# tensorflow/compression

Hardware: AMD Instinct MI355X
Metric: Mpixels/s encode+decode round-trip (bit-exact) (higher is better)
Workload: dtype int32

## Files before the change

### compression_amd/_lib.py

```python
from __future__ import annotations

import ctypes as C
import os

_HERE = os.path.dirname(os.path.abspath(__file__))
LIB_PATH = os.path.join(_HERE, "libtfc_hip.so")

_vp = C.c_void_p
_i64 = C.c_int64
_int = C.c_int

SIGNATURES = {
    "tfc_abi_version": (_int, []),
    "tfc_last_error": (C.c_char_p, []),
    "tfc_profile_enable": (None, [_int]),
    "tfc_set_default_mode": (_int, [_int]),
    "tfc_get_default_mode": (_int, []),
    "tfc_set_chip_shared": (_int, [_int]),
    "tfc_image_to_unit": (_int, [_vp, _vp, _int, C.c_int64, _vp]),
    "tfc_unit_to_image": (_int, [_vp, _int, _vp, C.c_int64, _vp]),
    "tfc_index_prepare": (_int, [_vp, _int, _vp, C.c_int64, _int, _vp]),
    "tfc_build_tables": (_int, [_vp, C.c_int64, C.c_int64, _vp, _vp, C.c_int64, _int, _vp, _vp]),
    "tfc_build_tables_overflow": (_int, [_vp, C.c_int64, C.c_int64, _vp, _vp, C.c_int64, _int, _vp, _vp, _vp]),
    "tfc_deep_factorized_tails": (_int, [_vp, C.c_int64, C.c_int64, _int, _int, _vp, _int, _vp, _vp, _vp]),
    "tfc_pad2d": (_int, [_vp, _vp, _int, C.c_int64, C.c_int64, C.c_int64, C.c_int64, _int, _int, _int, _int, _int, _vp]),
    "tfc_cache_bytes": (_int, [C.POINTER(C.c_longlong)]),
    "tfc_cache_trim": (_int, [C.POINTER(C.c_longlong)]),
    "tfc_encoder_capacity": (_int, [_vp, C.POINTER(_i64)]),
    "tfc_profile_query": (_int, [C.c_char_p, C.POINTER(C.c_double), C.POINTER(_i64)]),
    "tfc_pipe_counters": (_int, [C.POINTER(_i64), C.POINTER(_i64)]),
    "tfc_set_pipe_format": (_int, [_int, _int]),
    "tfc_tables_create": (_int, [_vp, _int, _i64, _i64, _vp, C.POINTER(_vp)]),
    "tfc_tables_count": (_i64, [_vp]),
    "tfc_tables_destroy": (None, [_vp]),
    "tfc_encoder_create": (_int, [_vp, _i64, _vp, C.POINTER(_vp)]),
    "tfc_encoder_create_many": (_int, [_vp, _i64, _int, _vp, _vp]),
    "tfc_encoder_set_mode": (_int, [_vp, _int]),
    "tfc_encoder_set_deferred_errors": (_int, [_vp, _int]),
    "tfc_encoder_encode": (_int, [_vp, _vp, _vp, _i64, _vp]),
    "tfc_encoder_encode_many": (_int, [_int, _vp, _vp, _vp, _i64, _vp]),
    "tfc_encoder_encode_quantized": (_int, [_vp, _vp, _int, _vp, _vp, _i64, _i64, _vp]),
    "tfc_encoder_encode_quantized_indexed": (_int, [_vp, _vp, _int, _vp, _vp, _i64, _vp]),
    "tfc_encoder_encode_quantized_many": (_int, [_int, _vp, _vp, _int, _vp, _vp, _i64, _i64, _vp]),
    "tfc_decoder_decode_dequantized_many": (_int, [_int, _vp, _vp, _int, _vp, _vp, _i64, _i64, _vp]),
    "tfc_encoder_encode_quantized_indexed_many": (_int, [_int, _vp, _vp, _int, _vp, _vp, _i64, _vp]),
    "tfc_decoder_decode_dequantized_indexed_many": (_int, [_int, _vp, _vp, _vp, _int, _vp, _i64, _vp]),
    "tfc_encoder_finalize": (_int, [_vp, _vp, C.POINTER(_i64)]),
    "tfc_encoder_finalize_device": (_int, [_vp, _vp]),
    "tfc_encoder_finalize_device_many": (_int, [_int, _vp, _vp]),
    "tfc_encoder_status": (_int, [_vp, _vp, C.POINTER(_i64)]),
    "tfc_encoder_result": (_int, [_vp, C.POINTER(_vp), C.POINTER(_vp)]),
    "tfc_encoder_read": (_int, [_vp, _vp, _vp, _int, _vp]),
    "tfc_encoder_destroy": (None, [_vp]),
    "tfc_decoder_create": (_int, [_vp, _vp, _vp, _i64, _int, _vp, C.POINTER(_vp)]),
    "tfc_decoder_create_many": (_int, [_vp, _int, _vp, _vp, _vp]),
    "tfc_decoder_set_mode": (_int, [_vp, _int]),
    "tfc_decoder_decode": (_int, [_vp, _vp, _vp, _i64, _vp]),
    "tfc_decoder_decode_many": (_int, [_int, _vp, _vp, _vp, _i64, _vp]),
    "tfc_decoder_decode_dequantized": (_int, [_vp, _vp, _vp, _int, _vp, _vp, _i64, _i64, _vp]),
    "tfc_decoder_finalize": (_int, [_vp, _vp, _vp]),
    "tfc_decoder_finalize_device": (_int, [_vp, _vp, _vp]),
    "tfc_decoder_finalize_device_many": (_int, [_int, _vp, _vp, _vp]),
    "tfc_decoder_status": (_int, [_vp, _vp]),
    "tfc_decoder_destroy": (None, [_vp]),
# ... 139 lines not shown
```

### compression_amd/csrc/range_coder.hip

```cpp
#include <hip/hip_bf16.h>
#include <hip/hip_fp16.h>
#include <hip/hip_runtime.h>

#include <algorithm>
#include <atomic>
#include <cstdlib>
#include <cstring>
#include <type_traits>
#include <memory>
#include <mutex>
#include <string>
#include <vector>

#include "../../include/tfc_hip.h"
#include "common.h"
#include "range_coder_device.h"
#include "range_tables.h"
#include "range_wave.h"

using namespace tfc;


namespace tfc {

// ... 530 lines not shown
  }
}
__global__ void fill_state_kernel(uint4* state, int64_t n, uint4 v, unsigned long long* status,
                                  unsigned int* oflag) {
  fill_state_one(state, n, v, status, oflag);
}
__global__ void fill_state_many_kernel(uint8_t* ctl, long long ctl_bytes, int64_t n, uint4 v) {
  uint8_t* c = ctl + blockIdx.y * ctl_bytes;
  fill_state_one(reinterpret_cast<uint4*>(c + 64), n, v, reinterpret_cast<unsigned long long*>(c),
                 reinterpret_cast<unsigned int*>(c + 32));
}

}


namespace {

int env_int(const char* name, int fallback) {
  const char* e = std::getenv(name);
  return e ? std::atoi(e) : fallback;
}

std::atomic<int>& pipe_format_value() {
  static std::atomic<int> v{[] {
    const char* e = std::getenv("TFC_PIPE_FORMAT");
    if (e && std::strcmp(e, "full") == 0) return 1;
    if (e && std::strcmp(e, "pairs") == 0) return 2;
    return 0;
  }()};
  return v;
}
std::atomic<int>& pipe_waves_value() {
  static std::atomic<int> v{std::max(0, env_int("TFC_PIPE_WAVES", 0))};
  return v;
}
inline int pipe_format() { return pipe_format_value().load(std::memory_order_relaxed); }
inline int pipe_waves_env() { return pipe_waves_value().load(std::memory_order_relaxed); }

inline bool pipe_enabled() {
  static const bool on = env_int("TFC_PIPE", 1) != 0;
  return on;
}
inline bool pipe_fallback_launch() {
  static const bool on = env_int("TFC_PIPE_NOFALLBACK", 0) == 0;
  return on;
}
std::atomic<long long>& pipe_launches() {
  static std::atomic<long long> n{0};
  return n;
}

inline int pipe_overlap() {
  static const int v = env_int("TFC_PIPE_OVERLAP", 2);
  return v;
}
inline long long pipe_poll_ticks() {
  static const long long v = static_cast<long long>(env_int("TFC_PIPE_POLL_MS", 250)) * 100000;
  return v;
}

struct SideStream {
  hipStream_t stream = nullptr;
  hipEvent_t fork = nullptr, join = nullptr;
};
inline int side_stream(hipStream_t st, SideStream* out) {
  static std::mutex mu;
// ... 233 lines not shown
    for (int k = 0; k < gn; ++k) {
      tfc_encoder* e = es[g0 + k];
      e->elems_last = elems;
      e->indexed_last = indexed;
      if (speculative && !e->deferred) {
        TFC_HIP(backups[g0 + k].alloc(sizeof(uint4) * streams, st));
        TFC_HIP(hipMemcpyAsync(backups[g0 + k].p, e->state.p, sizeof(uint4) * streams, hipMemcpyDeviceToDevice, st));
      }
      EncChunk ch;
      ch.stride = la.cap;
      ch.data_bytes = static_cast<size_t>(la.cap) * streams;
      TFC_HIP(ch.data.alloc(ch.data_bytes + sizeof(unsigned int) * streams, st));
      ch.len_p = reinterpret_cast<unsigned int*>(ch.data.as<uint8_t>() + ch.data_bytes);
      EncLaneJob<Src>& J = jobs.job[k];
      J.src = srcs[g0 + k];
      J.index = indexed ? indexes[g0 + k] : nullptr;
      J.state = e->state.as<uint4>();
      J.chunk = ch.data.as<uint8_t>();
      J.chunk_len = ch.len_p;
      J.first_error = e->status.as<unsigned long long>();
      J.overflow_flag = e->oflag.as<unsigned int>();
      errs.job[k].status = J.first_error;
      errs.job[k].src = J.src;
      errs.job[k].index = J.index;
      e->chunks.push_back(std::move(ch));
    }
    {
      KernelTimer timer("enc_kernel", st);
      DevBuf temp;
      bool piped = pipe;
      la.guard = nullptr;
      if (pipe) do {
        const size_t groups = static_cast<size_t>(pa.groups_per_job) * gn;
        const size_t calls_bytes = (groups * 64 * pa.rows + 64 * PipeEncChainLds::kRows) * sizeof(unsigned int);
        const size_t stage_bytes = groups * 64 * (sizeof(uint4) + sizeof(uint2));
        const size_t status_bytes = groups * pa.nt * 64 * sizeof(unsigned int);
        const size_t done_bytes = (groups * pa.nt * sizeof(unsigned int) + 255) & ~size_t{255};
        if (temp.alloc(calls_bytes + stage_bytes + status_bytes + done_bytes + 512, st) != hipSuccess) {
          (void)hipGetLastError();
          temp.p = nullptr;
          piped = false;
          break;
        }
        uint8_t* base = temp.as<uint8_t>();
        pa.calls = reinterpret_cast<unsigned int*>(base);
        pa.stage_state = reinterpret_cast<uint4*>(base + calls_bytes);
        pa.stage_out = reinterpret_cast<uint2*>(base + calls_bytes + groups * 64 * sizeof(uint4));
        pa.status = reinterpret_cast<unsigned int*>(base + calls_bytes + stage_bytes);
        pa.done = reinterpret_cast<unsigned int*>(base + calls_bytes + stage_bytes + status_bytes);
        pa.fallback = reinterpret_cast<unsigned int*>(base + calls_bytes + stage_bytes + status_bytes + done_bytes);
        pa.started = pa.fallback + 64;
        pa.groups = static_cast<int>(groups);
        pipe_launches().fetch_add(1, std::memory_order_relaxed);
        pa.fast16 = t->d_fast.as<uint16_t>();
        pa.rows_fast = t->d_rows_fast.as<int2>();
        pa.ntab = la.ntab;
        pa.tab_entries = t->host.size() * 2 <= static_cast<size_t>(kExpandTabBytes) ? static_cast<int>(t->host.size()) : 0;
        pa.cap = la.cap;
        TFC_HIP(hipMemsetAsync(pa.status, 0, status_bytes + done_bytes + 512, st));
        PipeChainJobs cj;
        cj.streams = streams;
        for (int k = 0; k < gn; ++k)
          cj.job[k] = PipeChainJob{jobs.job[k].state, jobs.job[k].chunk, jobs.job[k].chunk_len, jobs.job[k].overflow_flag};
        const bool large = groups >= 64;
        const int overlap = large ? pipe_overlap() : 0;
        SideStream side;
        if (overlap) {
          if (side_stream(st, &side)) return 1;
          TFC_HIP(hipEventRecord(side.fork, st));
          TFC_HIP(hipStreamWaitEvent(side.stream, side.fork, 0));
        }
        const hipStream_t cst = overlap ? side.stream : st;
        const dim3 xgrid(static_cast<unsigned>(groups * pa.nt));
        auto expand = [&] {
          KernelTimer t2("enc_expand", st);
          const bool tlds = pa.tab_entries != 0;
          if (indexed && tlds) hipLaunchKernelGGL((enc_expand_kernel<true, Src, true>), xgrid, dim3(kExpandThreads), 0, st, jobs, pa);
          else if (indexed) hipLaunchKernelGGL((enc_expand_kernel<true, Src, false>), xgrid, dim3(kExpandThreads), 0, st, jobs, pa);
          else if (tlds) hipLaunchKernelGGL((enc_expand_kernel<false, Src, true>), xgrid, dim3(kExpandThreads), 0, st, jobs, pa);
          else hipLaunchKernelGGL((enc_expand_kernel<false, Src, false>), xgrid, dim3(kExpandThreads), 0, st, jobs, pa);
        };
        const int cgroups = PipeEncChainLds::kGroups;
        const unsigned cblocks = static_cast<unsigned>(ceil_div(static_cast<int64_t>(groups), cgroups));
        const int clds = cgroups * PipeEncChainLds::kGroup;
        if (large)
          TFC_HIP(hipFuncSetAttribute(reinterpret_cast<const void*>(&enc_chain_kernel), hipFuncAttributeMaxDynamicSharedMemorySize, clds));
        auto chain = [&] {
          KernelTimer t2("enc_chain", cst);
          if (!large) {
            hipLaunchKernelGGL(enc_chain_direct_kernel, dim3(static_cast<unsigned>(groups)), dim3(64), 0, cst, cj, pa);
            return;
          }
          hipLaunchKernelGGL(enc_chain_kernel, dim3(cblocks), dim3(256 * cgroups), clds, cst, cj, pa);
          if (overlap == 2)
            hipLaunchKernelGGL(enc_gate_kernel, dim3(1), dim3(1), 0, st, pa.started, cblocks, static_cast<long long>(20000));
        };
        if (overlap == 2) { chain(); expand(); }
        else { expand(); chain(); }
        if (overlap) {
          TFC_HIP(hipEventRecord(side.join, side.stream));
          TFC_HIP(hipStreamWaitEvent(st, side.join, 0));
        }
        hipLaunchKernelGGL(enc_commit_kernel, dim3(static_cast<unsigned>(groups)), dim3(64), 0, st, cj, pa);
        la.guard = pa.fallback;
      } while (false);
      const dim3 grid(static_cast<unsigned>(jobs.blocks_per_job * gn));
      if (piped && !pipe_fallback_launch()) {}
      else if (indexed) hipLaunchKernelGGL((enc_lanes_kernel<true, Src>), grid, dim3(block), lds_bytes, st, jobs, la);
      else hipLaunchKernelGGL((enc_lanes_kernel<false, Src>), grid, dim3(block), lds_bytes, st, jobs, la);
    }
    hipLaunchKernelGGL((enc_error_kernel<Src>), dim3(1), dim3(64), 0, st, errs);
    TFC_HIP(hipGetLastError());
  }
  bool any_eager = false;
  for (int k = 0; k < n; ++k) any_eager |= !es[k]->deferred;
  if (any_eager) {
    TFC_HIP(hipStreamSynchronize(st));
    for (int k = 0; k < n; ++k) {
      tfc_encoder* e = es[k];
      if (e->deferred) continue;
      unsigned long long host_status[4];
      TFC_HIP(hipMemcpy(host_status, e->status.p, sizeof(host_status), hipMemcpyDeviceToHost));
      if (host_status[0] != ~0ull) return encoder_error(e, host_status);
      if (!speculative) continue;
      unsigned int oflag = 0;
      TFC_HIP(hipMemcpy(&oflag, e->oflag.p, sizeof(oflag), hipMemcpyDeviceToHost));
// ... 378 lines not shown
  for (int k = 0; k < n; ++k) {
    tfc_encoder* e = es[k];
    e->result_group = group;
    e->offsets.p = f.base + k * f.job_bytes + f.offsets_off;
    e->blob.p = f.base + k * f.job_bytes + f.blob_off;
    e->blob_capacity = static_cast<int64_t>(cap);
    e->chunks.clear();
    e->finalized = true;
  }
  return 0;
}

extern "C" int tfc_debug_pipe_clocks(unsigned long long* out8) {
  TFC_HIP(hipDeviceSynchronize());
  TFC_HIP(hipMemcpyFromSymbol(out8, HIP_SYMBOL(tfc::g_pipe_clock), 8 * sizeof(unsigned long long)));
  return 0;
}
extern "C" int tfc_debug_enc_clocks(unsigned long long* out4) {
  TFC_HIP(hipDeviceSynchronize());
  TFC_HIP(hipMemcpyFromSymbol(out4, HIP_SYMBOL(tfc::g_enc_clock), 4 * sizeof(unsigned long long)));
  return 0;
}

extern "C" int tfc_pipe_counters(int64_t* launches, int64_t* fallback_blocks) {
  if (launches) *launches = pipe_launches().load();
  if (fallback_blocks) {
    unsigned long long v = 0;
    TFC_HIP(hipDeviceSynchronize());
    TFC_HIP(hipMemcpyFromSymbol(&v, HIP_SYMBOL(tfc::g_pipe_fallback_blocks), sizeof(v)));
    *fallback_blocks = static_cast<int64_t>(v);
  }
  return 0;
}

extern "C" int tfc_set_pipe_format(int format, int waves_per_workgroup) {
  if (format < 0 || format > 2 || waves_per_workgroup < 0 || waves_per_workgroup > 8) {
    tfc::fail("tfc_set_pipe_format: format 0 ... 2, waves per workgroup 0 ... 8");
    return -1;
  }
  pipe_waves_value().store(waves_per_workgroup);
  return pipe_format_value().exchange(format);
}

extern "C" int tfc_encoder_set_mode(tfc_encoder* e, int mode) {
  if (mode != TFC_MODE_AUTO && mode != TFC_MODE_LATENCY && mode != TFC_MODE_THROUGHPUT)
    return fail("unknown mode %d", mode);
  if (e->family >= 0) return fail("the mode of a handle is fixed by its first coding call");
  e->mode = mode;
  return 0;
}

extern "C" int tfc_encoder_set_deferred_errors(tfc_encoder* e, int on) {
  e->deferred = on != 0;
  return 0;
}

extern "C" int tfc_encoder_encode(tfc_encoder* e, const int32_t* value, const int32_t* index,
                                  int64_t elems, void* stream) {
  const SymInt32 src{value};
  return encode_jobs(&e, 1, &src, &index, elems, static_cast<hipStream_t>(stream), "tfc_encoder_encode");
}

extern "C" int tfc_encoder_encode_many(int n, tfc_encoder* const* es, const int32_t* const* values,
                                       const int32_t* const* indexes, int64_t elems, void* stream) {
  if (n <= 0) return 0;
  std::vector<SymInt32> srcs(n);
// ... 722 lines not shown
```

### compression_amd/csrc/range_pipe.h

```cpp
#pragma once

#ifndef TFC_PIPE_TIMING
#define TFC_PIPE_TIMING 0
#endif

namespace tfc {

constexpr int kPipeTile = 256;
constexpr int kPipeEscMax = 32;
constexpr unsigned int kPipeBlock = 16;
constexpr unsigned int kPipeNoCall = 0x0001FFFFu;
constexpr unsigned int kPipeAggregate = 1u << 30;
constexpr unsigned int kPipePrefix = 2u << 30;
constexpr unsigned int kPipeRowsMask = (1u << 30) - 1u;

struct PipeEncArgs {
  const uint16_t* fast16;
  const int2* rows_fast;
  int ntab;
  int tab_entries;
  unsigned int* calls;
  unsigned int* status;
  unsigned int* done;
  unsigned int* fallback;
  unsigned int* started;
  uint4* stage_state;
  uint2* stage_out;
  int nt;
  int rows;
  int groups_per_job;
  int groups;
  unsigned int cap;
  long long poll_ticks;
};


__device__ inline unsigned int pipe_escape_extra(unsigned int g) { return 2u * static_cast<unsigned int>(31 - __clz(static_cast<int>(g))) + 2u; }
__device__ inline unsigned int pipe_escape_word(unsigned int g, unsigned int neg, unsigned int extra, unsigned int k) {
  const unsigned int left = extra - k;
  const unsigned int sft = left - 1u;
  const unsigned int bit = left == 0u ? neg : (sft < 32u ? (g >> sft) & 1u : 0u);
  return bit ? 0x00008000u : 0x80000000u;
}

constexpr int kExpandThreads = 512;
constexpr int kExpandTabBytes = 32 * 1024;
template <bool INDEXED, typename Src, bool TABLDS>
__global__ void __launch_bounds__(kExpandThreads, 4) enc_expand_kernel(const EncLaneJobs<Src> jobs, const PipeEncArgs pa) {
  constexpr int kRow = kPipeTile;
  constexpr int kHalves = kExpandThreads / kPipeTile;
  __shared__ unsigned short W[64 * kRow];
  __shared__ __attribute__((aligned(16))) unsigned short tab[kExpandTabBytes / 2];
  __shared__ unsigned int esc[64][kPipeEscMax];
  __shared__ unsigned short ecum[64][kPipeEscMax];
  __shared__ unsigned int ecount[64], nesc[64], start[64];

  const unsigned int gi = blockIdx.x % static_cast<unsigned int>(pa.groups);
  const unsigned int T = blockIdx.x / static_cast<unsigned int>(pa.groups);
  const unsigned int job = gi / static_cast<unsigned int>(pa.groups_per_job);
  const unsigned int gidx = gi % static_cast<unsigned int>(pa.groups_per_job);
  const EncLaneJob<Src>& J = jobs.job[job];
  const Src src = J.src;
  const int32_t* const index = J.index;
  const unsigned int tid = threadIdx.x, lane = tid & 63u;
  const unsigned int elems = static_cast<unsigned int>(jobs.elems);
  const int64_t s0 = static_cast<int64_t>(gidx) * 64;
  const unsigned int ntab = static_cast<unsigned int>(pa.ntab);
  if (tid < 64u) ecount[tid] = 0u;
  constexpr bool tab_lds = TABLDS;
  if (tab_lds) {
    const uint4* const src16 = reinterpret_cast<const uint4*>(pa.fast16);
    for (unsigned int i = tid; i < (static_cast<unsigned int>(pa.tab_entries) + 7u) / 8u; i += kExpandThreads)
      reinterpret_cast<uint4*>(tab)[i] = src16[i];
  }
  __syncthreads();

  auto escape_of = [&](int64_t s, unsigned int at, unsigned int& g, unsigned int& neg) {
    const int64_t pos = s * jobs.elems + at;
    int t = static_cast<int>(at % ntab);
    if (INDEXED) {
      t = tfc_gload(index + pos);
      if (t < 0 || t >= pa.ntab) t = 0;
    }
    const int2 row = pa.rows_fast[t];
    const int32_t v = src.load(pos, t);
    const int32_t vmax = (row.y & 0x7FFFFFFF) - 3;
    neg = v < 0 ? 1u : 0u;
    g = v < 0 ? 0u - static_cast<unsigned int>(v) : static_cast<unsigned int>(v - vmax) + 1u;
  };

  {
    constexpr int N = 64 / kHalves;
    constexpr int NB = INDEXED ? 8 : 16;
    const unsigned int p = tid % kPipeTile, half = tid / kPipeTile;
    const unsigned int j = T * kPipeTile + p;
    const bool inpos = j < elems;
    const unsigned int jc = inpos ? j : 0u;
    const int tch = static_cast<int>(jc % ntab);
    const int2 rowc = pa.rows_fast[tch];
    unsigned long long badpos = ~0ull;
    auto position = [&](int i) {
      const int64_t s = s0 + i * kHalves + static_cast<int>(half);
// ... 80 lines not shown
    __hip_atomic_store(st + static_cast<size_t>(T) * 64, kPipeAggregate | cnt, __ATOMIC_RELAXED, __HIP_MEMORY_SCOPE_AGENT);
    unsigned int before = 0u;
    bool stuck = false;
    long long t0 = 0;
    for (unsigned int t = T; t-- > 0u && !stuck;) {
      unsigned int v, spins = 0u;
      while (((v = __hip_atomic_load(st + static_cast<size_t>(t) * 64, __ATOMIC_RELAXED, __HIP_MEMORY_SCOPE_AGENT)) >> 30) == 0u) {
        if (++spins < 64u) continue;
        __builtin_amdgcn_s_sleep(16);
        const long long now = static_cast<long long>(wall_clock64());
        if (t0 == 0) t0 = now;
        else if (now - t0 > pa.poll_ticks) { stuck = true; break; }
      }
      if (stuck) break;
      before += v & kPipeRowsMask;
      if (v & kPipePrefix) break;
    }
    const unsigned int limit = static_cast<unsigned int>(pa.rows);
    const bool fits = !stuck && before + cnt <= limit;
    if (!fits) atomicOr(&pa.fallback[job], 1u);
    __hip_atomic_store(st + static_cast<size_t>(T) * 64, kPipePrefix | (fits ? before + cnt : limit + 1u), __ATOMIC_RELAXED,
                       __HIP_MEMORY_SCOPE_AGENT);
    start[tid] = fits ? before : 0xFFFFFFFFu;
  }
  __syncthreads();

  {
    constexpr unsigned int kWaves = kExpandThreads / 64;
    const unsigned int q = tid >> 6;
    for (unsigned int sl = q; sl < 64u; sl += kWaves) {
      const unsigned int first = start[sl];
      if (first == 0xFFFFFFFFu || s0 + sl >= jobs.streams) continue;
      unsigned int* const gbase = pa.calls + static_cast<size_t>(gi) * 64 * pa.rows;
      auto out = [&](unsigned int r) -> unsigned int& {
        return gbase[((static_cast<size_t>(r >> 5) * 64 + sl) << 5) + (r & 31u)];
      };
      const unsigned int ne = nesc[sl];
      for (unsigned int p = lane; p < valid; p += 64u) {
        unsigned int cum = 0u;
        for (unsigned int i = 0; i < ne; ++i) {
          const unsigned int e = esc[sl][i];
          cum += (e & 0xFFu) < p ? (e >> 9) & 0x7Fu : 0u;
        }
        const unsigned int at = W[sl * kRow + p];
        unsigned int word;
        if constexpr (tab_lds) word = static_cast<unsigned int>(tab[at]) | (static_cast<unsigned int>(tab[at + 1u]) << 16);
        else word = reinterpret_cast<const TFC_AS1 LanePacked<unsigned int>*>((const TFC_AS1 void*)(pa.fast16 + at))->v;
#ifndef TFC_EXPAND_INFLIGHT
#define TFC_EXPAND_INFLIGHT 1
#endif
        asm volatile("s_waitcnt vmcnt(%0)" ::"n"(TFC_EXPAND_INFLIGHT) : "memory");
        out(first + p + cum) = word;
      }
      if (lane < ne) {
        const unsigned int e = esc[sl][lane];
        const unsigned int epos = e & 0xFFu, neg = (e >> 8) & 1u, extra = (e >> 9) & 0x7Fu;
        unsigned int g = e >> 16, ng;
        if (extra >= 34u) escape_of(s0 + sl, T * kPipeTile + epos, g, ng);
        const unsigned int row = epos + ecum[sl][lane];
        for (unsigned int k = 1; k <= extra; ++k) out(first + row + k) = pipe_escape_word(g, neg, extra, k);
      }
    }
  }
  __syncthreads();
  if (tid == 0) __hip_atomic_store(&pa.done[static_cast<size_t>(gi) * pa.nt + T], 1u, __ATOMIC_RELEASE, __HIP_MEMORY_SCOPE_AGENT);
}


#define TFC_PENC_ROW(W)                                                                    \
  "v_cmpx_ne_u32 vcc, %[NOCALL], %[" #W "]\n\t"                                            \
  "v_and_b32 v100, %[KFFFF], %[" #W "]\n\t"                                                \
  "v_lshrrev_b32 v102, 16, %[" #W "]\n\t"                                                  \
  "v_mad_u64_u32 v[104:105], s[52:53], v100, %[S], v[100:101]\n\t"                         \
  "v_mad_u64_u32 v[106:107], s[52:53], v102, %[S], v[102:103]\n\t"                         \
  "v_alignbit_b32 v104, v105, v104, 16\n\t"                                               \
  "v_alignbit_b32 v106, v107, v106, 16\n\t"                                               \
  "v_add_u32 v106, -1, v106\n\t"                                                          \
  "v_min_u32 v106, v106, %[S]\n\t"                                                        \
  "v_add_co_u32 v108, vcc, %[BASE], v104\n\t"                                             \
  "v_addc_co_u32 v111, vcc, 0, %[H], vcc\n\t"                                             \
  "v_sub_u32 v109, v106, v104\n\t"                                                        \
  "v_sub_u32 v117, v111, %[H]\n\t"                                                        \
  "v_cmp_gt_u32 vcc, %[K64K], v109\n\t"                                                   \
  "v_cndmask_b32 v118, 0, 1, vcc\n\t"
#define TFC_PENC_STEP(W)                                                                   \
  TFC_PENC_ROW(W)                                                                          \
  "v_perm_b32 v110, 0, v111, %[PERM]\n\t"                                                 \
  "ds_write_b16 %[NA], v110\n\t"                                                          \
  "v_or_b32 v112, v117, v118\n\t"                                                         \
  "v_and_b32 v112, v112, %[HAD]\n\t"                                                      \
  "v_lshl_add_u32 %[NA], v112, 1, %[NA]\n\t"                                              \
  "v_lshrrev_b32 v113, 16, v108\n\t"                                                      \
  "v_lshlrev_b32 v114, 16, v108\n\t"                                                      \
  "v_lshl_or_b32 v115, v109, 16, %[KFFFF]\n\t"                                            \
  "v_cndmask_b32 %[BASE], v108, v114, vcc\n\t"                                            \
  "v_cndmask_b32 %[S], v109, v115, vcc\n\t"                                               \
  "v_cndmask_b32 %[H], %[H], v113, vcc\n\t"                                               \
  "v_or_b32 v119, %[HAD], v118\n\t"                                                       \
  "v_bfi_b32 %[HAD], v117, v118, v119\n\t"                                                \
  "v_cmp_eq_u32 vcc, %[KFFFF], %[H]\n\t"                                                  \
  "v_addc_co_u32 %[FLAG], vcc, 0, %[FLAG], vcc\n\t"
#define TFC_PENC_STEP_H(W)                                                                 \
  "v_cmpx_ne_u32 vcc, %[NOCALL], %[" #W "]\n\t"                                            \
  "v_and_b32 v100, %[KFFFF], %[" #W "]\n\t"                                                \
  "v_lshrrev_b32 v102, 16, %[" #W "]\n\t"                                                  \
  "v_mad_u64_u32 v[104:105], s[52:53], v100, %[S], v[100:101]\n\t"                         \
  "v_mad_u64_u32 v[106:107], s[52:53], v102, %[S], v[102:103]\n\t"                         \
  "v_alignbit_b32 v104, v105, v104, 16\n\t"                                               \
  "v_alignbit_b32 v106, v107, v106, 16\n\t"                                               \
  "v_add_u32 v106, -1, v106\n\t"                                                          \
  "v_min_u32 v106, v106, %[S]\n\t"                                                        \
  "v_add_co_u32 v108, vcc, %[BASE], v104\n\t"                                             \
  "v_addc_co_u32 v111, vcc, 0, %[H], vcc\n\t"                                             \
  "v_sub_u32 v109, v106, v104\n\t"                                                        \
  "v_cmp_gt_u32 vcc, %[K64K], v109\n\t"                                                   \
  "ds_write_b16 %[NA], v111\n\t"                                                          \
  "v_cndmask_b32 v112, 0, %[HAD], vcc\n\t"                                                \
  "v_add_u32 %[NA], %[NA], v112\n\t"                                                      \
  "v_cndmask_b32 %[HAD], %[HAD], v119, vcc\n\t"                                           \
  "v_lshlrev_b32 v114, 16, v108\n\t"                                                      \
  "v_lshl_or_b32 v115, v109, 16, %[KFFFF]\n\t"                                            \
  "v_cndmask_b32 %[BASE], v108, v114, vcc\n\t"                                            \
  "v_cndmask_b32 %[S], v109, v115, vcc\n\t"                                               \
  "v_cndmask_b32_sdwa %[H], v111, v108, vcc dst_sel:DWORD dst_unused:UNUSED_PAD src0_sel:DWORD src1_sel:WORD_1\n\t" \
  "v_cmpx_gt_u32 vcc, %[KFFFF], %[H]\n\t"

struct PipeEncChainLds {
  static constexpr unsigned int kRows = 2 * kPipeBlock;
#ifndef TFC_ENC_SLOTS
#define TFC_ENC_SLOTS 4
#endif
  static constexpr unsigned int kSlots = TFC_ENC_SLOTS;
#ifndef TFC_ENC_DIGSLOTS
#define TFC_ENC_DIGSLOTS 6
#endif
  static constexpr unsigned int kDigSlots = TFC_ENC_DIGSLOTS;
  static constexpr unsigned int kDigits = 2 * kRows + 16;
  static constexpr int kCallStride = 4 * kRows + 16;
  static constexpr int kCallSlot = 64 * kCallStride;
  static constexpr int kDigStride = lane_stride(kDigits + 8);
  static constexpr int kDigSlot = 64 * kDigStride;
  static constexpr int kCalls = 0;
  static constexpr int kDig = kCalls + kSlots * kCallSlot;
  static constexpr int kRec = kDig + kDigSlots * kDigSlot;
  static constexpr int kSync = kRec + kDigSlots * 64 * 8;
  static constexpr int kGroup = kSync + 64;
#ifndef TFC_ENC_GROUPS
#define TFC_ENC_GROUPS 2
#endif
  static constexpr int kGroups = TFC_ENC_GROUPS;
  static constexpr int kSeq = 0;
  static constexpr int kConsumed = 4;
  static constexpr int kDigPub = 5;
  static constexpr int kDigDone = 6;
  static constexpr int kExit = 7;
  static constexpr unsigned int kLast = 0x80000000u, kBail = 0x40000000u;
};
static_assert(PipeEncChainLds::kGroups * PipeEncChainLds::kGroup <= 160 * 1024 && PipeEncChainLds::kSlots <= 4, "a chain workgroup's LDS");
struct PipeChainJob { uint4* state; uint8_t* chunk; unsigned int* chunk_len; unsigned int* overflow_flag; };
struct PipeChainJobs {
  int64_t streams;
  PipeChainJob job[64];
};

__global__ void __launch_bounds__(1024) enc_chain_kernel(const PipeChainJobs jobs, const PipeEncArgs pa) {
  using L = PipeEncChainLds;
  constexpr unsigned int kRows = L::kRows;
  extern __shared__ __attribute__((aligned(16))) unsigned char chain_lds[];
  const unsigned int G = blockDim.x >> 8;
  if (threadIdx.x == 0u) __hip_atomic_fetch_add(pa.started, 1u, __ATOMIC_RELAXED, __HIP_MEMORY_SCOPE_AGENT);
  for (unsigned int i = threadIdx.x; i < G * 16u; i += blockDim.x)
    reinterpret_cast<unsigned int*>(chain_lds + (i / 16u) * L::kGroup + L::kSync)[i % 16u] = 0u;
  __syncthreads();

  const unsigned int wave = threadIdx.x >> 6, lane = threadIdx.x & 63u;
  const unsigned int gi = blockIdx.x * G + (wave % G);
  if (gi >= static_cast<unsigned int>(pa.groups)) return;
  const unsigned int role = wave / G;
  unsigned char* const area = chain_lds + (wave % G) * L::kGroup;
  typedef __attribute__((address_space(3))) unsigned int lds_u32;
  volatile lds_u32* const sync = reinterpret_cast<volatile lds_u32*>(
      (__attribute__((address_space(3))) unsigned char*)chain_lds + (wave % G) * L::kGroup + L::kSync);
  const unsigned int area_off = static_cast<unsigned int>(reinterpret_cast<size_t>((__attribute__((address_space(3))) unsigned char*)area));

  const unsigned int job = gi / static_cast<unsigned int>(pa.groups_per_job);
  const unsigned int gidx = gi % static_cast<unsigned int>(pa.groups_per_job);
  const PipeChainJob& J = jobs.job[job];
  const int64_t s = static_cast<int64_t>(gidx) * 64 + lane;
  const bool live = s < jobs.streams;
  unsigned char* const out = J.chunk + (live ? s : 0) * static_cast<int64_t>(pa.cap);

  if (role == 1u || role == 2u) {
    const unsigned int nt = static_cast<unsigned int>(pa.nt);
    const unsigned int* const status = pa.status + static_cast<size_t>(gi) * nt * 64 + lane;
    const unsigned int* const done = pa.done + static_cast<size_t>(gi) * nt;
    const unsigned char* const words = reinterpret_cast<const unsigned char*>(pa.calls + static_cast<size_t>(gi) * 64 * pa.rows);
    unsigned int avail = 0u;
    unsigned int tn = 0u;
    bool bail = __hip_atomic_load(&pa.fallback[job], __ATOMIC_RELAXED, __HIP_MEMORY_SCOPE_AGENT) != 0u;
    auto ensure = [&](unsigned int need) {
      while (tn < nt && __any(live && avail < need)) {
        const unsigned int* const flag = done + tn;
        long long t0 = 0;
        bool timing = false;
        while (__hip_atomic_load(flag, __ATOMIC_RELAXED, __HIP_MEMORY_SCOPE_AGENT) == 0u) {
          const long long now = static_cast<long long>(wall_clock64());
          if (!timing) { t0 = now; timing = true; }
          else if (now - t0 > pa.poll_ticks) { bail = true; return; }
          __builtin_amdgcn_s_sleep(8);
        }
        __builtin_amdgcn_fence(__ATOMIC_ACQUIRE, "agent");
        avail = __hip_atomic_load(status + static_cast<size_t>(tn) * 64, __ATOMIC_RELAXED, __HIP_MEMORY_SCOPE_AGENT) & kPipeRowsMask;
        ++tn;
        if (__hip_atomic_load(&pa.fallback[job], __ATOMIC_RELAXED, __HIP_MEMORY_SCOPE_AGENT) != 0u) { bail = true; return; }
      }
    };
    for (unsigned int b = role - 1u;; b += 2u) {
      const unsigned int slot = b % L::kSlots;
      if (!bail) ensure((b + 1u) * kRows);
      if (!bail && tn == nt && !__any(b * kRows < avail)) break;
      uint4 v[kRows / 4u];
      if (!bail) {
        const unsigned char* const p = words + static_cast<size_t>(b) * (64u * kRows * 4u) + 16u * lane;
#pragma unroll
        for (unsigned int c = 0; c < kRows / 4u; ++c) v[c] = lanes_gload16(p + 1024u * c);
        if (__any(avail < (b + 1u) * kRows)) {
          const unsigned int r0 = b * kRows + 4u * (lane & 7u);
#pragma unroll
          for (unsigned int c = 0; c < kRows / 4u; ++c) {
            const unsigned int theirs = static_cast<unsigned int>(__shfl(static_cast<int>(avail), static_cast<int>(8u * c + (lane >> 3))));
            v[c].x = r0 + 0u < theirs ? v[c].x : kPipeNoCall;
            v[c].y = r0 + 1u < theirs ? v[c].y : kPipeNoCall;
            v[c].z = r0 + 2u < theirs ? v[c].z : kPipeNoCall;
            v[c].w = r0 + 3u < theirs ? v[c].w : kPipeNoCall;
          }
        }
      }
      bool gone = false;
      while (b >= sync[L::kConsumed] + L::kSlots) {
        if (sync[L::kExit] != 0u) { gone = true; break; }
        __builtin_amdgcn_s_sleep(2);
      }
      if (gone) break;
      if (bail) {
        if (lane == 0u) {
          sync[L::kSeq + slot] = L::kBail;
          atomicOr(&pa.fallback[job], 1u);
        }
        break;
      }
#pragma unroll
      for (unsigned int c = 0; c < kRows / 4u; ++c)
        *reinterpret_cast<uint4*>(area + L::kCalls + slot * L::kCallSlot + L::kCallStride * (8u * c + (lane >> 3)) + 16u * (lane & 7u)) = v[c];
      const bool last = tn == nt && !__any((b + 1u) * kRows < avail);
      asm volatile("s_waitcnt lgkmcnt(0)" ::: "memory");
      if (lane == 0u) sync[L::kSeq + slot] = (b + 1u) | (last ? L::kLast : 0u);
      if (last) break;
    }
    return;
  }

  if (role == 3u) {
    for (unsigned int b_store = 0u;;) {
      if (b_store < sync[L::kDigPub]) {
        const unsigned int ds = b_store % L::kDigSlots;
        const uint2 rec = reinterpret_cast<const uint2*>(area + L::kRec)[ds * 64u + lane];
        const unsigned char* const src = area + L::kDig + ds * L::kDigSlot + L::kDigStride * lane;
        unsigned char* const dst = out + rec.x;
#pragma unroll
        for (unsigned int c = 0; c < L::kDigits / 16u; ++c) {
          if (16u * c < rec.y && rec.x + 16u * c + 16u <= pa.cap) {
            uint2 lo = reinterpret_cast<const uint2*>(src)[2 * c], hi = reinterpret_cast<const uint2*>(src)[2 * c + 1];
            lo.x = __builtin_amdgcn_perm(lo.x, lo.x, 0x02030001u); lo.y = __builtin_amdgcn_perm(lo.y, lo.y, 0x02030001u);
            hi.x = __builtin_amdgcn_perm(hi.x, hi.x, 0x02030001u); hi.y = __builtin_amdgcn_perm(hi.y, hi.y, 0x02030001u);
            lanes_gstore16(dst + 16u * c, lo, hi);
          }
        }
        ++b_store;
        asm volatile("s_waitcnt lgkmcnt(0)" ::: "memory");
        if (lane == 0u) sync[L::kDigDone] = b_store;
      } else {
        if (sync[L::kExit] != 0u && b_store == sync[L::kDigPub]) break;
        __builtin_amdgcn_s_sleep(2);
      }
    }
    return;
// ... 1207 lines not shown
```

### include/tfc_hip.h

```cpp
#ifndef TFC_HIP_H_
#define TFC_HIP_H_

#include <stdint.h>

#ifdef __cplusplus
extern "C" {
#endif

typedef struct tfc_tables tfc_tables;
typedef struct tfc_encoder tfc_encoder;
typedef struct tfc_decoder tfc_decoder;

#define TFC_ABI_VERSION 2
int tfc_abi_version(void);
const char* tfc_last_error(void);

void tfc_profile_enable(int on);
int tfc_profile_query(const char* kernel, double* total_ms, int64_t* launches);
int tfc_pipe_counters(int64_t* launches, int64_t* fallback_blocks);
int tfc_set_pipe_format(int format, int waves_per_workgroup);

#define TFC_MODE_AUTO 0
#define TFC_MODE_LATENCY 1
#define TFC_MODE_THROUGHPUT 2
int tfc_set_default_mode(int mode);
int tfc_get_default_mode(void);

int tfc_set_chip_shared(int shared);
int tfc_image_to_unit(const void* x, void* y, int dtype, int64_t n, void* stream);
int tfc_unit_to_image(const void* x, int dtype, void* y, int64_t n, void* stream);
int tfc_index_prepare(const void* indexes, int dtype, int32_t* out, int64_t n, int num_tables, void* stream);
int tfc_pad2d(const void* x, void* y, int elem_bytes, int64_t n, int64_t h, int64_t w, int64_t c, int top, int bottom,
              int left, int right, int reflect, void* stream);
int tfc_cache_bytes(long long* bytes);
int tfc_cache_trim(long long* released);


int tfc_tables_create(const int32_t* lookup, int rank, int64_t rows, int64_t cols,
                      void* stream, tfc_tables** out);
int64_t tfc_tables_count(const tfc_tables* t);
void tfc_tables_destroy(tfc_tables* t);


int tfc_encoder_create(const tfc_tables* tables, int64_t streams, void* stream,
                       tfc_encoder** out);

int tfc_encoder_create_many(const tfc_tables* tables, int64_t streams, int n, void* stream,
                            tfc_encoder** out);

int tfc_encoder_set_mode(tfc_encoder* e, int mode);
int tfc_encoder_set_deferred_errors(tfc_encoder* e, int on);

int tfc_encoder_encode(tfc_encoder* e, const int32_t* value, const int32_t* index,
// ... 294 lines not shown
```

Baseline: 62050.

## Store 16-bit call codes in global memory and expand via LDS table in chain kernel

The expand kernel now writes 16-bit table indices (plus escape-bit codes) to the global call buffer instead of 32-bit packed call words. The chain kernel loads the code table into LDS and expands each code into its 32-bit word when filling its call slots. This halves the global traffic between expand and chain kernels. In exchange it adds table staging, an extra LDS gather per call, fewer LDS call slots (3 instead of 4) and a new template path. It is enabled by default for large launches whose table fits.

```diff
diff --git a/compression_amd/_lib.py b/compression_amd/_lib.py
--- a/compression_amd/_lib.py
+++ b/compression_amd/_lib.py
@@ -30,6 +30,8 @@
     "tfc_profile_query": (_int, [C.c_char_p, C.POINTER(C.c_double), C.POINTER(_i64)]),
     "tfc_pipe_counters": (_int, [C.POINTER(_i64), C.POINTER(_i64)]),
     "tfc_set_pipe_format": (_int, [_int, _int]),
+    "tfc_set_pipe_calls": (_int, [_int]),
+    "tfc_pipe_calls_last": (_int, []),
     "tfc_tables_create": (_int, [_vp, _int, _i64, _i64, _vp, C.POINTER(_vp)]),
     "tfc_tables_count": (_i64, [_vp]),
     "tfc_tables_destroy": (None, [_vp]),
diff --git a/compression_amd/csrc/range_coder.hip b/compression_amd/csrc/range_coder.hip
--- a/compression_amd/csrc/range_coder.hip
+++ b/compression_amd/csrc/range_coder.hip
@@ -586,6 +586,17 @@
 }
 std::atomic<int>& pipe_waves_value() {
   static std::atomic<int> v{std::max(0, env_int("TFC_PIPE_WAVES", 0))};
+  return v;
+}
+std::atomic<int>& pipe_calls_value() {
+  static std::atomic<int> v{[] {
+    const int e = env_int("TFC_PIPE_CALLS", 0);
+    return e == 16 || e == 32 ? e : 0;
+  }()};
+  return v;
+}
+std::atomic<int>& pipe_calls_last() {
+  static std::atomic<int> v{0};
   return v;
 }
 inline int pipe_format() { return pipe_format_value().load(std::memory_order_relaxed); }
@@ -885,7 +896,13 @@
       la.guard = nullptr;
       if (pipe) do {
         const size_t groups = static_cast<size_t>(pa.groups_per_job) * gn;
-        const size_t calls_bytes = (groups * 64 * pa.rows + 64 * PipeEncChainLds::kRows) * sizeof(unsigned int);
+        const bool large = groups >= 64;
+        pa.tab_entries = t->host.size() * 2 <= static_cast<size_t>(kExpandTabBytes) ? static_cast<int>(t->host.size()) : 0;
+        const bool calls16 = large && pa.tab_entries != 0 && pipe_calls_value().load(std::memory_order_relaxed) != 32 &&
+                             pipe_code_image_bytes(pa.tab_entries) <= PipeEncChainLds16::kImageBytes &&
+                             t->host.size() + kPipeCodeExtra <= 65536;
+        const size_t calls_bytes = calls16 ? groups * 64 * pipe_rows16(pa.rows) * sizeof(unsigned short)
+                                           : (groups * 64 * pa.rows + 64 * PipeEncChainLds::kRows) * sizeof(unsigned int);
         const size_t stage_bytes = groups * 64 * (sizeof(uint4) + sizeof(uint2));
         const size_t status_bytes = groups * pa.nt * 64 * sizeof(unsigned int);
         const size_t done_bytes = (groups * pa.nt * sizeof(unsigned int) + 255) & ~size_t{255};
@@ -905,17 +922,16 @@
         pa.started = pa.fallback + 64;
         pa.groups = static_cast<int>(groups);
         pipe_launches().fetch_add(1, std::memory_order_relaxed);
+        pipe_calls_last().store(calls16 ? 16 : 32, std::memory_order_relaxed);
         pa.fast16 = t->d_fast.as<uint16_t>();
         pa.rows_fast = t->d_rows_fast.as<int2>();
         pa.ntab = la.ntab;
-        pa.tab_entries = t->host.size() * 2 <= static_cast<size_t>(kExpandTabBytes) ? static_cast<int>(t->host.size()) : 0;
         pa.cap = la.cap;
         TFC_HIP(hipMemsetAsync(pa.status, 0, status_bytes + done_bytes + 512, st));
         PipeChainJobs cj;
         cj.streams = streams;
         for (int k = 0; k < gn; ++k)
           cj.job[k] = PipeChainJob{jobs.job[k].state, jobs.job[k].chunk, jobs.job[k].chunk_len, jobs.job[k].overflow_flag};
-        const bool large = groups >= 64;
         const int overlap = large ? pipe_overlap() : 0;
         SideStream side;
         if (overlap) {
@@ -928,23 +944,27 @@
         auto expand = [&] {
           KernelTimer t2("enc_expand", st);
           const bool tlds = pa.tab_entries != 0;
-          if (indexed && tlds) hipLaunchKernelGGL((enc_expand_kernel<true, Src, true>), xgrid, dim3(kExpandThreads), 0, st, jobs, pa);
+          if (calls16 && indexed) hipLaunchKernelGGL((enc_expand_kernel<true, Src, true, true>), xgrid, dim3(kExpandThreads), 0, st, jobs, pa);
+          else if (calls16) hipLaunchKernelGGL((enc_expand_kernel<false, Src, true, true>), xgrid, dim3(kExpandThreads), 0, st, jobs, pa);
+          else if (indexed && tlds) hipLaunchKernelGGL((enc_expand_kernel<true, Src, true>), xgrid, dim3(kExpandThreads), 0, st, jobs, pa);
           else if (indexed) hipLaunchKernelGGL((enc_expand_kernel<true, Src, false>), xgrid, dim3(kExpandThreads), 0, st, jobs, pa);
           else if (tlds) hipLaunchKernelGGL((enc_expand_kernel<false, Src, true>), xgrid, dim3(kExpandThreads), 0, st, jobs, pa);
           else hipLaunchKernelGGL((enc_expand_kernel<false, Src, false>), xgrid, dim3(kExpandThreads), 0, st, jobs, pa);
         };
         const int cgroups = PipeEncChainLds::kGroups;
         const unsigned cblocks = static_cast<unsigned>(ceil_div(static_cast<int64_t>(groups), cgroups));
-        const int clds = cgroups * PipeEncChainLds::kGroup;
+        const int clds = calls16 ? cgroups * PipeEncChainLds16::kGroup + pipe_code_image_bytes(pa.tab_entries) : cgroups * PipeEncChainLds::kGroup;
         if (large)
-          TFC_HIP(hipFuncSetAttribute(reinterpret_cast<const void*>(&enc_chain_kernel), hipFuncAttributeMaxDynamicSharedMemorySize, clds));
+          TFC_HIP(hipFuncSetAttribute(calls16 ? reinterpret_cast<const void*>(&enc_chain_kernel<true>) : reinterpret_cast<const void*>(&enc_chain_kernel<false>),
+                                      hipFuncAttributeMaxDynamicSharedMemorySize, clds));
         auto chain = [&] {
           KernelTimer t2("enc_chain", cst);
           if (!large) {
             hipLaunchKernelGGL(enc_chain_direct_kernel, dim3(static_cast<unsigned>(groups)), dim3(64), 0, cst, cj, pa);
             return;
           }
-          hipLaunchKernelGGL(enc_chain_kernel, dim3(cblocks), dim3(256 * cgroups), clds, cst, cj, pa);
+          if (calls16) hipLaunchKernelGGL(enc_chain_kernel<true>, dim3(cblocks), dim3(256 * cgroups), clds, cst, cj, pa);
+          else hipLaunchKernelGGL(enc_chain_kernel<false>, dim3(cblocks), dim3(256 * cgroups), clds, cst, cj, pa);
           if (overlap == 2)
             hipLaunchKernelGGL(enc_gate_kernel, dim3(1), dim3(1), 0, st, pa.started, cblocks, static_cast<long long>(20000));
         };
@@ -1389,6 +1409,16 @@
   }
   return 0;
 }
+
+extern "C" int tfc_set_pipe_calls(int bits) {
+  if (bits != 0 && bits != 16 && bits != 32) {
+    tfc::fail("tfc_set_pipe_calls: 0 (by launch), 16 or 32");
+    return -1;
+  }
+  return pipe_calls_value().exchange(bits);
+}
+
+extern "C" int tfc_pipe_calls_last(void) { return pipe_calls_last().load(); }
 
 extern "C" int tfc_set_pipe_format(int format, int waves_per_workgroup) {
   if (format < 0 || format > 2 || waves_per_workgroup < 0 || waves_per_workgroup > 8) {
diff --git a/compression_amd/csrc/range_pipe.h b/compression_amd/csrc/range_pipe.h
--- a/compression_amd/csrc/range_pipe.h
+++ b/compression_amd/csrc/range_pipe.h
@@ -36,21 +36,26 @@
 
 
 __device__ inline unsigned int pipe_escape_extra(unsigned int g) { return 2u * static_cast<unsigned int>(31 - __clz(static_cast<int>(g))) + 2u; }
-__device__ inline unsigned int pipe_escape_word(unsigned int g, unsigned int neg, unsigned int extra, unsigned int k) {
+__device__ inline unsigned int pipe_escape_bit(unsigned int g, unsigned int neg, unsigned int extra, unsigned int k) {
   const unsigned int left = extra - k;
   const unsigned int sft = left - 1u;
-  const unsigned int bit = left == 0u ? neg : (sft < 32u ? (g >> sft) & 1u : 0u);
-  return bit ? 0x00008000u : 0x80000000u;
+  return left == 0u ? neg : (sft < 32u ? (g >> sft) & 1u : 0u);
 }
+__device__ inline unsigned int pipe_escape_word(unsigned int g, unsigned int neg, unsigned int extra, unsigned int k) {
+  return pipe_escape_bit(g, neg, extra, k) ? 0x00008000u : 0x80000000u;
+}
+__host__ __device__ inline unsigned int pipe_rows16(unsigned int rows) { return (rows + 63u) & ~63u; }
+constexpr unsigned int kPipeCodeExtra = 5;
+constexpr unsigned int kPipeCodeNoCall = 3;
 
 constexpr int kExpandThreads = 512;
 constexpr int kExpandTabBytes = 32 * 1024;
-template <bool INDEXED, typename Src, bool TABLDS>
+template <bool INDEXED, typename Src, bool TABLDS, bool CALLS16 = false>
 __global__ void __launch_bounds__(kExpandThreads, 4) enc_expand_kernel(const EncLaneJobs<Src> jobs, const PipeEncArgs pa) {
   constexpr int kRow = kPipeTile;
   constexpr int kHalves = kExpandThreads / kPipeTile;
   __shared__ unsigned short W[64 * kRow];
-  __shared__ __attribute__((aligned(16))) unsigned short tab[kExpandTabBytes / 2];
+  __shared__ __attribute__((aligned(16))) unsigned short tab[TABLDS && !CALLS16 ? kExpandTabBytes / 2 : 8];
   __shared__ unsigned int esc[64][kPipeEscMax];
   __shared__ unsigned short ecum[64][kPipeEscMax];
   __shared__ unsigned int ecount[64], nesc[64], start[64];
@@ -67,7 +72,7 @@
   const int64_t s0 = static_cast<int64_t>(gidx) * 64;
   const unsigned int ntab = static_cast<unsigned int>(pa.ntab);
   if (tid < 64u) ecount[tid] = 0u;
-  constexpr bool tab_lds = TABLDS;
+  constexpr bool tab_lds = TABLDS && !CALLS16;
   if (tab_lds) {
     const uint4* const src16 = reinterpret_cast<const uint4*>(pa.fast16);
     for (unsigned int i = tid; i < (static_cast<unsigned int>(pa.tab_entries) + 7u) / 8u; i += kExpandThreads)
@@ -214,8 +219,12 @@
       const unsigned int first = start[sl];
       if (first == 0xFFFFFFFFu || s0 + sl >= jobs.streams) continue;
       unsigned int* const gbase = pa.calls + static_cast<size_t>(gi) * 64 * pa.rows;
+      unsigned short* const gbase16 = reinterpret_cast<unsigned short*>(pa.calls) + static_cast<size_t>(gi) * 64 * pipe_rows16(pa.rows);
       auto out = [&](unsigned int r) -> unsigned int& {
         return gbase[((static_cast<size_t>(r >> 5) * 64 + sl) << 5) + (r & 31u)];
+      };
+      auto out16 = [&](unsigned int r) -> unsigned short& {
+        return gbase16[((static_cast<size_t>(r >> 6) * 64 + sl) << 6) + (r & 63u)];
       };
       const unsigned int ne = nesc[sl];
       for (unsigned int p = lane; p < valid; p += 64u) {
@@ -225,14 +234,16 @@
           cum += (e & 0xFFu) < p ? (e >> 9) & 0x7Fu : 0u;
         }
         const unsigned int at = W[sl * kRow + p];
-        unsigned int word;
-        if constexpr (tab_lds) word = static_cast<unsigned int>(tab[at]) | (static_cast<unsigned int>(tab[at + 1u]) << 16);
+        unsigned int word = at;
+        if constexpr (CALLS16) {}
+        else if constexpr (tab_lds) word = static_cast<unsigned int>(tab[at]) | (static_cast<unsigned int>(tab[at + 1u]) << 16);
         else word = reinterpret_cast<const TFC_AS1 LanePacked<unsigned int>*>((const TFC_AS1 void*)(pa.fast16 + at))->v;
 #ifndef TFC_EXPAND_INFLIGHT
 #define TFC_EXPAND_INFLIGHT 1
 #endif
         asm volatile("s_waitcnt vmcnt(%0)" ::"n"(TFC_EXPAND_INFLIGHT) : "memory");
-        out(first + p + cum) = word;
+        if constexpr (CALLS16) out16(first + p + cum) = static_cast<unsigned short>(word);
+        else out(first + p + cum) = word;
       }
       if (lane < ne) {
         const unsigned int e = esc[sl][lane];
@@ -240,7 +251,11 @@
         unsigned int g = e >> 16, ng;
         if (extra >= 34u) escape_of(s0 + sl, T * kPipeTile + epos, g, ng);
         const unsigned int row = epos + ecum[sl][lane];
-        for (unsigned int k = 1; k <= extra; ++k) out(first + row + k) = pipe_escape_word(g, neg, extra, k);
+        const unsigned int bit0 = static_cast<unsigned int>(pa.tab_entries);
+        for (unsigned int k = 1; k <= extra; ++k) {
+          if constexpr (CALLS16) out16(first + row + k) = static_cast<unsigned short>(bit0 + pipe_escape_bit(g, neg, extra, k));
+          else out(first + row + k) = pipe_escape_word(g, neg, extra, k);
+        }
       }
     }
   }
@@ -307,12 +322,16 @@
   "v_cndmask_b32_sdwa %[H], v111, v108, vcc dst_sel:DWORD dst_unused:UNUSED_PAD src0_sel:DWORD src1_sel:WORD_1\n\t" \
   "v_cmpx_gt_u32 vcc, %[KFFFF], %[H]\n\t"
 
-struct PipeEncChainLds {
+template <unsigned int SLOTS>
+struct PipeEncChainLdsT {
   static constexpr unsigned int kRows = 2 * kPipeBlock;
 #ifndef TFC_ENC_SLOTS
 #define TFC_ENC_SLOTS 4
 #endif
-  static constexpr unsigned int kSlots = TFC_ENC_SLOTS;
+#ifndef TFC_ENC_SLOTS16
+#define TFC_ENC_SLOTS16 3
+#endif
+  static constexpr unsigned int kSlots = SLOTS;
 #ifndef TFC_ENC_DIGSLOTS
 #define TFC_ENC_DIGSLOTS 6
 #endif
@@ -337,22 +356,46 @@
   static constexpr int kDigDone = 6;
   static constexpr int kExit = 7;
   static constexpr unsigned int kLast = 0x80000000u, kBail = 0x40000000u;
+  static constexpr int kImageBytes = 160 * 1024 - kGroups * kGroup;
 };
+using PipeEncChainLds = PipeEncChainLdsT<TFC_ENC_SLOTS>;
+using PipeEncChainLds16 = PipeEncChainLdsT<TFC_ENC_SLOTS16>;
 static_assert(PipeEncChainLds::kGroups * PipeEncChainLds::kGroup <= 160 * 1024 && PipeEncChainLds::kSlots <= 4, "a chain workgroup's LDS");
+static_assert(PipeEncChainLds16::kImageBytes >= 26 * 1024 && PipeEncChainLds16::kSlots <= 4 && PipeEncChainLds16::kSlots >= 2,
+              "a chain workgroup's LDS, 16-bit call codes: two groups and BASELINE config 2's 25 KB image");
+static_assert(PipeEncChainLds16::kGroups == PipeEncChainLds::kGroups && PipeEncChainLds16::kRows == PipeEncChainLds::kRows, "one launch plan");
+__host__ __device__ constexpr int pipe_code_image_bytes(int entries) { return ((entries + static_cast<int>(kPipeCodeExtra) + 7) / 8) * 16; }
 struct PipeChainJob { uint4* state; uint8_t* chunk; unsigned int* chunk_len; unsigned int* overflow_flag; };
 struct PipeChainJobs {
   int64_t streams;
   PipeChainJob job[64];
 };
 
+template <bool CALLS16>
 __global__ void __launch_bounds__(1024) enc_chain_kernel(const PipeChainJobs jobs, const PipeEncArgs pa) {
-  using L = PipeEncChainLds;
+  using L = PipeEncChainLdsT<CALLS16 ? TFC_ENC_SLOTS16 : TFC_ENC_SLOTS>;
   constexpr unsigned int kRows = L::kRows;
   extern __shared__ __attribute__((aligned(16))) unsigned char chain_lds[];
   const unsigned int G = blockDim.x >> 8;
   if (threadIdx.x == 0u) __hip_atomic_fetch_add(pa.started, 1u, __ATOMIC_RELAXED, __HIP_MEMORY_SCOPE_AGENT);
   for (unsigned int i = threadIdx.x; i < G * 16u; i += blockDim.x)
     reinterpret_cast<unsigned int*>(chain_lds + (i / 16u) * L::kGroup + L::kSync)[i % 16u] = 0u;
+  typedef __attribute__((address_space(3))) unsigned short lds_u16;
+  const lds_u16* const img = reinterpret_cast<const lds_u16*>((__attribute__((address_space(3))) unsigned char*)chain_lds + G * L::kGroup);
+  const unsigned int nent = static_cast<unsigned int>(pa.tab_entries);
+  if constexpr (CALLS16) {
+    const uint4* const src16 = reinterpret_cast<const uint4*>(pa.fast16);
+    for (unsigned int i = threadIdx.x; i < (nent + 7u) / 8u; i += blockDim.x)
+      reinterpret_cast<uint4*>(chain_lds + G * L::kGroup)[i] = lanes_gload16(src16 + i);
+    __syncthreads();
+    if (threadIdx.x < kPipeCodeExtra) {
+      constexpr unsigned short kExtra[kPipeCodeExtra] = {0u, 0x8000u, 0u, 0xFFFFu, 0x0001u};
+      unsigned short v = kExtra[0];
+#pragma unroll
+      for (unsigned int k = 1; k < kPipeCodeExtra; ++k) v = threadIdx.x == k ? kExtra[k] : v;
+      reinterpret_cast<unsigned short*>(chain_lds + G * L::kGroup)[nent + threadIdx.x] = v;
+    }
+  }
   __syncthreads();
 
   const unsigned int wave = threadIdx.x >> 6, lane = threadIdx.x & 63u;
@@ -377,6 +420,7 @@
     const unsigned int* const status = pa.status + static_cast<size_t>(gi) * nt * 64 + lane;
     const unsigned int* const done = pa.done + static_cast<size_t>(gi) * nt;
     const unsigned char* const words = reinterpret_cast<const unsigned char*>(pa.calls + static_cast<size_t>(gi) * 64 * pa.rows);
+    const unsigned char* const words16 = reinterpret_cast<const unsigned char*>(pa.calls) + static_cast<size_t>(gi) * 64 * pipe_rows16(pa.rows) * 2u;
     unsigned int avail = 0u;
     unsigned int tn = 0u;
     bool bail = __hip_atomic_load(&pa.fallback[job], __ATOMIC_RELAXED, __HIP_MEMORY_SCOPE_AGENT) != 0u;
@@ -401,20 +445,41 @@
       const unsigned int slot = b % L::kSlots;
       if (!bail) ensure((b + 1u) * kRows);
       if (!bail && tn == nt && !__any(b * kRows < avail)) break;
-      uint4 v[kRows / 4u];
+      constexpr unsigned int kReq = CALLS16 ? kRows / 8u : kRows / 4u;
+      uint4 v[kReq];
       if (!bail) {
-        const unsigned char* const p = words + static_cast<size_t>(b) * (64u * kRows * 4u) + 16u * lane;
-#pragma unroll
-        for (unsigned int c = 0; c < kRows / 4u; ++c) v[c] = lanes_gload16(p + 1024u * c);
-        if (__any(avail < (b + 1u) * kRows)) {
-          const unsigned int r0 = b * kRows + 4u * (lane & 7u);
-#pragma unroll
-          for (unsigned int c = 0; c < kRows / 4u; ++c) {
-            const unsigned int theirs = static_cast<unsigned int>(__shfl(static_cast<int>(avail), static_cast<int>(8u * c + (lane >> 3))));
-            v[c].x = r0 + 0u < theirs ? v[c].x : kPipeNoCall;
-            v[c].y = r0 + 1u < theirs ? v[c].y : kPipeNoCall;
-            v[c].z = r0 + 2u < theirs ? v[c].z : kPipeNoCall;
-            v[c].w = r0 + 3u < theirs ? v[c].w : kPipeNoCall;
+        if constexpr (CALLS16) {
+          const unsigned char* const p = words16 + static_cast<size_t>(b >> 1) * (64u * 2u * kRows * 2u) + (b & 1u) * (2u * kRows) +
+                                         128u * (lane >> 2) + 16u * (lane & 3u);
+#pragma unroll
+          for (unsigned int c = 0; c < kReq; ++c) v[c] = lanes_gload16(p + 2048u * c);
+          if (__any(avail < (b + 1u) * kRows)) {
+            const unsigned int r0 = b * kRows + 8u * (lane & 3u);
+            const unsigned int nc = nent + kPipeCodeNoCall, nc2 = nc | (nc << 16);
+#pragma unroll
+            for (unsigned int c = 0; c < kReq; ++c) {
+              const unsigned int theirs = static_cast<unsigned int>(__shfl(static_cast<int>(avail), static_cast<int>(16u * c + (lane >> 2))));
+              auto pad = [&](unsigned int& h, unsigned int r) {
+                const unsigned int keep = (r < theirs ? 0x0000FFFFu : 0u) | (r + 1u < theirs ? 0xFFFF0000u : 0u);
+                h = (h & keep) | (nc2 & ~keep);
+              };
+              pad(v[c].x, r0); pad(v[c].y, r0 + 2u); pad(v[c].z, r0 + 4u); pad(v[c].w, r0 + 6u);
+            }
+          }
+        } else {
+          const unsigned char* const p = words + static_cast<size_t>(b) * (64u * kRows * 4u) + 16u * lane;
+#pragma unroll
+          for (unsigned int c = 0; c < kReq; ++c) v[c] = lanes_gload16(p + 1024u * c);
+          if (__any(avail < (b + 1u) * kRows)) {
+            const unsigned int r0 = b * kRows + 4u * (lane & 7u);
+#pragma unroll
+            for (unsigned int c = 0; c < kReq; ++c) {
+              const unsigned int theirs = static_cast<unsigned int>(__shfl(static_cast<int>(avail), static_cast<int>(8u * c + (lane >> 3))));
+              v[c].x = r0 + 0u < theirs ? v[c].x : kPipeNoCall;
+              v[c].y = r0 + 1u < theirs ? v[c].y : kPipeNoCall;
+              v[c].z = r0 + 2u < theirs ? v[c].z : kPipeNoCall;
+              v[c].w = r0 + 3u < theirs ? v[c].w : kPipeNoCall;
+            }
           }
         }
       }
@@ -431,9 +496,26 @@
         }
         break;
       }
-#pragma unroll
-      for (unsigned int c = 0; c < kRows / 4u; ++c)
-        *reinterpret_cast<uint4*>(area + L::kCalls + slot * L::kCallSlot + L::kCallStride * (8u * c + (lane >> 3)) + 16u * (lane & 7u)) = v[c];
+      if constexpr (CALLS16) {
+        const unsigned int cmax = nent + kPipeCodeNoCall;
+#pragma unroll
+        for (unsigned int c = 0; c < kReq; ++c) {
+          const unsigned int h[4] = {v[c].x, v[c].y, v[c].z, v[c].w};
+          unsigned int w[8];
+#pragma unroll
+          for (unsigned int k = 0; k < 8u; ++k) {
+            const unsigned int code = min((k & 1u) ? h[k >> 1] >> 16 : h[k >> 1] & 0xFFFFu, cmax);
+            w[k] = static_cast<unsigned int>(img[code]) | (static_cast<unsigned int>(img[code + 1u]) << 16);
+          }
+          uint4* const dst = reinterpret_cast<uint4*>(area + L::kCalls + slot * L::kCallSlot + L::kCallStride * (16u * c + (lane >> 2)) + 32u * (lane & 3u));
+          dst[0] = make_uint4(w[0], w[1], w[2], w[3]);
+          dst[1] = make_uint4(w[4], w[5], w[6], w[7]);
+        }
+      } else {
+#pragma unroll
+        for (unsigned int c = 0; c < kReq; ++c)
+          *reinterpret_cast<uint4*>(area + L::kCalls + slot * L::kCallSlot + L::kCallStride * (8u * c + (lane >> 3)) + 16u * (lane & 7u)) = v[c];
+      }
       const bool last = tn == nt && !__any((b + 1u) * kRows < avail);
       asm volatile("s_waitcnt lgkmcnt(0)" ::: "memory");
       if (lane == 0u) sync[L::kSeq + slot] = (b + 1u) | (last ? L::kLast : 0u);
diff --git a/include/tfc_hip.h b/include/tfc_hip.h
--- a/include/tfc_hip.h
+++ b/include/tfc_hip.h
@@ -19,6 +19,8 @@
 int tfc_profile_query(const char* kernel, double* total_ms, int64_t* launches);
 int tfc_pipe_counters(int64_t* launches, int64_t* fallback_blocks);
 int tfc_set_pipe_format(int format, int waves_per_workgroup);
+int tfc_set_pipe_calls(int bits);
+int tfc_pipe_calls_last(void);
 
 #define TFC_MODE_AUTO 0
 #define TFC_MODE_LATENCY 1
```

Result: slower. 60450 (-2.6%).
